# ShuhangGu/DASR

Hardware: NVIDIA B200
Metric: x4 SR output megapixels/sec (RRDBNet-23 G forward) (higher is better)
Workload: dtype bf16

## Files before the change

dasr_b200/csrc/conv_tc2.cu:

```cuda
#include <stdlib.h>
#include "tc_common.cuh"

namespace dasr {

constexpr int TC2_EPI_WARPS = 8;
constexpr int TC2_WARPS = 2 + TC2_EPI_WARPS + 1;
constexpr int TC2_THREADS = 32 * TC2_WARPS;
constexpr int TC2_MAX_STAGES = 6;
constexpr int TC2_MAX_BLOCKS = 6;

struct Tc2Maps {
  CUtensorMap m[8];
};

struct Tc2Args {
  DasrConvTcParams p;
  const float* bias;
  int nchunks;
  int n_half;
  int tiles_x, tiles_y;
  long ntiles;
  int stages, a_stage_bytes, w_bytes;
  int nblk;
  int nb64;
  int nb;
  int acc_stride;
};

template <bool HAS_PRE, int NRES>
__global__ void __cluster_dims__(2, 1, 1) __launch_bounds__(TC2_THREADS, 1)
conv_tc2_kernel(const __grid_constant__ CUtensorMap tmap_in, const __grid_constant__ CUtensorMap tmap_w,
                const __grid_constant__ Tc2Maps em, const Tc2Args a) {
  extern __shared__ __align__(1024) uint8_t smem_raw[];
  uint8_t* smem = reinterpret_cast<uint8_t*>((reinterpret_cast<uintptr_t>(smem_raw) + 1023) & ~uintptr_t(1023));
  uint8_t* sW = smem;
  uint8_t* sA = smem + a.w_bytes;
  uint8_t* sS = sA + (size_t)a.stages * a.a_stage_bytes;
  uint8_t* sR1 = sS + (size_t)a.nblk * EPI_BLK64_BYTES;
  uint8_t* sR2 = sR1 + (NRES >= 1 ? (size_t)a.nblk * EPI_BLK64_BYTES : 0);
  uint64_t* bars = reinterpret_cast<uint64_t*>(sR2 + (NRES >= 2 ? (size_t)a.nblk * EPI_BLK64_BYTES : 0));
  constexpr bool HAS_LOADS = HAS_PRE || NRES > 0;
  uint64_t* full_bar = bars;
  uint64_t* empty_bar = bars + TC2_MAX_STAGES;
  uint64_t* w_bar = bars + 2 * TC2_MAX_STAGES;
  uint64_t* tfull_bar = w_bar + 1;
  uint64_t* tempty_bar = tfull_bar + 2;
  uint64_t* sfull_bar = tempty_bar + 2;
  uint64_t* sfree_bar = sfull_bar + TC2_MAX_BLOCKS;
  uint64_t* pre_bar = sfree_bar + TC2_MAX_BLOCKS;
  uint32_t* tmem_ptr = reinterpret_cast<uint32_t*>(pre_bar + TC2_MAX_BLOCKS);
  float* sBias = reinterpret_cast<float*>(bars + 40);

  const DasrConvTcParams& p = a.p;
  const int warp = threadIdx.x >> 5, lane = threadIdx.x & 31;
  const uint32_t rank = cluster_ctarank();
  const long pair = blockIdx.x >> 1, npairs = gridDim.x >> 1;
  const int cout = p.nt;
  const int co_base = (int)blockIdx.y * p.nt;

  if (threadIdx.x == 0) {
    tma_prefetch_desc(&tmap_in);
    tma_prefetch_desc(&tmap_w);
    tma_prefetch_desc(&em.m[0]);
    for (int s = 0; s < a.stages; s++) {
      mbar_init(&full_bar[s], 1);
      mbar_init(&empty_bar[s], 1);
    }
    mbar_init(w_bar, 1);
    for (int b = 0; b < 2; b++) {
      mbar_init(&tfull_bar[b], 1);
      mbar_init(&tempty_bar[b], 2 * TC2_EPI_WARPS);
    }
    for (int b = 0; b < a.nblk; b++) {
      mbar_init(&sfull_bar[b], TC2_EPI_WARPS);
      mbar_init(&sfree_bar[b], 1);
      mbar_init(&pre_bar[b], 1);
    }
    fence_barrier_init();
  }
  for (int i = threadIdx.x; i < cout; i += TC2_THREADS) sBias[i] = a.bias ? a.bias[co_base + i] : 0.f;
  cluster_sync();
  if (warp == 1) tmem_alloc2(tmem_ptr, 512);
  tc_fence_before();
  __syncthreads();
  tc_fence_after();
  const uint32_t tmem_base = *tmem_ptr;
  pdl_launch_dependents();

  auto tile_of = [&](long it, int& x0, int& y0, int& n) -> bool {
    uint32_t t = 2u * (uint32_t)(pair + it * npairs) + rank;
    const bool live = (long)t < a.ntiles;
    if (p.tile_rev && live) t = (uint32_t)(a.ntiles - 1) - t;
    const uint32_t r = t / (uint32_t)a.tiles_x;
    const uint32_t tx = t - r * (uint32_t)a.tiles_x;
    n = (int)(r / (uint32_t)a.tiles_y);
    const uint32_t ty = r - (uint32_t)n * (uint32_t)a.tiles_y;
    x0 = (int)tx * TILE_W;
    y0 = (int)ty * TILE_H;
    return live;
  };
  const long niter = (a.ntiles / 2 + (a.ntiles & 1) - pair + npairs - 1) / npairs;

  if (warp == 0) {
    if (lane == 0) {
      if (rank == 0) mbar_expect_tx(w_bar, 2u * (uint32_t)a.w_bytes);
      for (int tap = 0; tap < 9; tap++)
        for (int c = 0; c < a.nchunks; c++) {
          const int slot = tap * a.nchunks + c;
          const int row = slot * p.cout + co_base + (int)rank * a.n_half;
          tma2_load_2d(sW + (size_t)slot * a.n_half * ROW_B, &tmap_w, w_bar, 0, row);
        }
      pdl_wait();
      int stage = 0;
      uint32_t phase = 0;
      for (long it = 0; it < niter; it++) {
        int x0, y0, n;
        tile_of(it, x0, y0, n);
        for (int c = 0; c < a.nchunks; c++) {
          mbar_wait(&empty_bar[stage], phase ^ 1);
          if (rank == 0) mbar_expect_tx(&full_bar[stage], 2u * A_HALO_BYTES);
          tma2_load_4d(sA + (size_t)stage * a.a_stage_bytes, &tmap_in, &full_bar[stage],
                       p.nchunk_list ? p.chunk_off[c] : p.in_coff + c * CHUNK, x0 - 1, y0 - 1, n);
          if (++stage == a.stages) { stage = 0; phase ^= 1; }
        }
      }
    }
    __syncwarp();
  } else if (warp == 1) {
    if (rank == 0) {
      const uint32_t idesc = make_idesc_16(256, cout, p.f16);
      const uint32_t a_sbo = (uint32_t)(HALO_W * ROW_B);
      const uint64_t a_hi = ((uint64_t)((a_sbo >> 4) & 0x3FFF) << 32) | ((uint64_t)1 << 46) | ((uint64_t)4 << 61) | ((uint64_t)1 << 16);
      const uint64_t b_hi = ((uint64_t)(((8 * ROW_B) >> 4) & 0x3FFF) << 32) | ((uint64_t)1 << 46) | ((uint64_t)4 << 61) | ((uint64_t)1 << 16);
      const uint32_t a_lo0 = smem_u32(sA) >> 4;
      const uint32_t a_stage_lo = (uint32_t)a.a_stage_bytes >> 4;
      const uint32_t b_lo0 = smem_u32(sW) >> 4;
      const uint32_t b_slot_lo = (uint32_t)(a.n_half * ROW_B) >> 4;
      uint32_t tap_lo[9];
#pragma unroll
      for (int t = 0; t < 9; t++) tap_lo[t] = (uint32_t)(((t / 3) * HALO_W + (t % 3)) * ROW_B) >> 4;
      mbar_wait(w_bar, 0);
      tc_fence_after();
      int stage = 0;
      uint32_t phase = 0;
      for (long it = 0; it < niter; it++) {
        const int acc = (int)(it & 1);
        mbar_wait(&tempty_bar[acc], ((uint32_t)(it >> 1) & 1) ^ 1);
        tc_fence_after();
        const uint32_t d_tmem = tmem_base + (uint32_t)(acc * a.acc_stride);
        for (int c = 0; c < a.nchunks; c++) {
          mbar_wait(&full_bar[stage], phase);
          tc_fence_after();
          if (elect_one()) {
            const uint32_t a_lo = a_lo0 + (uint32_t)stage * a_stage_lo;
            uint32_t b_lo = b_lo0 + (uint32_t)c * b_slot_lo;
            const uint32_t b_tap_step = (uint32_t)a.nchunks * b_slot_lo;
#pragma unroll
            for (int tap = 0; tap < 9; tap++) {
              const uint32_t al = a_lo + tap_lo[tap];
              umma2_bf16(d_tmem, a_hi | (uint64_t)(al & 0x3FFF), b_hi | (uint64_t)(b_lo & 0x3FFF), idesc, (uint32_t)((c | tap) != 0));
              umma2_bf16(d_tmem, a_hi | (uint64_t)((al + 2) & 0x3FFF), b_hi | (uint64_t)((b_lo + 2) & 0x3FFF), idesc, 1u);
              b_lo += b_tap_step;
            }
            umma2_commit_mc(&empty_bar[stage]);
            if (c == a.nchunks - 1) umma2_commit_mc(&tfull_bar[acc]);
          }
          __syncwarp();
          if (++stage == a.stages) { stage = 0; phase ^= 1; }
        }
      }
    }
  } else if (warp == TC2_WARPS - 1) {
    if (lane == 0) {
      pdl_wait();
      const uint32_t nb = (uint32_t)a.nb, nblk = (uint32_t)a.nblk;
      const uint32_t total = (uint32_t)niter * nb;
      const uint32_t nld = (uint32_t)((HAS_PRE ? 1 : 0) + NRES);
      const bool mask_mode = (NRES >= 1) && (p.mask_c1 > p.mask_c0);
      auto issue_loads = [&](uint32_t k) {
        const uint32_t b = k % nblk;
        int x0, y0, n;
        const uint32_t kt = k / nb;
        tile_of((long)kt, x0, y0, n);
        const int i = (int)(k - kt * nb);
        const int wide = i < a.nb64 ? 1 : 0;
        const int col = co_base + i * 64;
        const bool need_r1 = !mask_mode || (col < p.mask_c1 && col + (wide ? 64 : 32) > p.mask_c0);
        mbar_expect_tx(&pre_bar[b], (nld - (need_r1 ? 0u : 1u)) * (uint32_t)(wide ? EPI_BLK64_BYTES : EPI_BLK32_BYTES));
        if constexpr (HAS_PRE) tma_load_4d(sS + (size_t)b * EPI_BLK64_BYTES, &em.m[wide ? 2 : 3], &pre_bar[b], p.pre_coff + col, x0, y0, n);
        if constexpr (NRES >= 1) {
          if (need_r1) tma_load_4d(sR1 + (size_t)b * EPI_BLK64_BYTES, &em.m[wide ? 4 : 5], &pre_bar[b], p.res1_coff + col, x0, y0, n);
        }
        if constexpr (NRES >= 2) tma_load_4d(sR2 + (size_t)b * EPI_BLK64_BYTES, &em.m[wide ? 6 : 7], &pre_bar[b], p.res2_coff + col, x0, y0, n);
      };
      if constexpr (HAS_LOADS)
        for (uint32_t k = 0; k < nblk && k < total; k++) issue_loads(k);
      auto retire = [&](uint32_t k) {
        if constexpr (HAS_LOADS) {
          if (k + nblk < total) issue_loads(k + nblk);
        } else {
          mbar_arrive(&sfree_bar[k % nblk]);
        }
      };
      int x0 = 0, y0 = 0, n = 0;
      bool live = false;
      uint32_t i = 0;
      for (uint32_t k = 0; k < total; k++) {
        const uint32_t b = k % nblk;
        if (i == 0) live = tile_of((long)(k / nb), x0, y0, n);
        mbar_wait(&sfull_bar[b], (k / nblk) & 1);
        if (live) tma_store_4d(&em.m[(int)i < a.nb64 ? 0 : 1], sS + (size_t)b * EPI_BLK64_BYTES, p.out_coff + co_base + (int)i * 64, x0, y0, n);
        bulk_commit();
        if (k >= 1) {
          asm volatile("cp.async.bulk.wait_group.read 1;" ::: "memory");
          retire(k - 1);
        }
        if (++i == nb) i = 0;
      }
      if (total > 0) {
        bulk_wait_read0();
        retire(total - 1);
      }
      bulk_wait0();
    }
    __syncwarp();
  } else {
    const int ew = warp - 2;
    const int wg = ew >> 2;
    const int q = warp & 3;
    const int m = q * 32 + lane;
    const int sw128 = m & 7, sw64 = (m >> 1) & 3;
    const int act = p.act, f16 = p.f16;
    const float slope = p.slope, alpha = p.alpha;
    const bool scale = alpha != 1.f;
    const uint32_t sS_u = smem_u32(sS), sR1_u = smem_u32(sR1), sR2_u = smem_u32(sR2), sBias_u = smem_u32(sBias);
    const bool has_bias = a.bias != nullptr;
    uint32_t k = 0;
    for (long it = 0; it < niter; it++) {
      const int acc = (int)(it & 1);
      mbar_wait(&tfull_bar[acc], (uint32_t)(it >> 1) & 1);
      tc_fence_after();
      const uint32_t t_addr = tmem_base + ((uint32_t)(q * 32) << 16) + (uint32_t)(acc * a.acc_stride);
      for (int i = 0; i < a.nb; i++, k++) {
        const int b = (int)(k % (uint32_t)a.nblk);
        if constexpr (HAS_LOADS) {
          mbar_wait(&pre_bar[b], (k / (uint32_t)a.nblk) & 1);
        } else {
          if (k >= (uint32_t)a.nblk) mbar_wait(&sfree_bar[b], ((k / (uint32_t)a.nblk) & 1) ^ 1);
// ... 62 lines not shown
#pragma unroll
                for (int j = 0; j < 8; j++) {
                  if (!(ms0[j] > 0)) v[j] *= p.mask_slope;
                  if (!(ms1[j] > 0)) v[8 + j] *= p.mask_slope;
                }
              }
            } else {
              fma_h16x8(v, lds128(bR1 + o0), p.beta1, f16);
              fma_h16x8(v + 8, lds128(bR1 + o1), p.beta1, f16);
            }
          }
          if constexpr (NRES >= 2) {
            fma_h16x8(v, lds128(bR2 + o0), p.beta2, f16);
            fma_h16x8(v + 8, lds128(bR2 + o1), p.beta2, f16);
          }
          uint4 o[2];
          pack_h16x16(v, o, f16);
          sts128(bS + o0, o[0]);
          sts128(bS + o1, o[1]);
        }
        fence_proxy_async();
        __syncwarp();
        if (lane == 0) mbar_arrive(&sfull_bar[b]);
      }
    }
  }

  tc_fence_before();
  cluster_sync();
  if (warp == 1) {
    tc_fence_after();
    tmem_dealloc2(tmem_base, 512);
  }
}

__global__ void __cluster_dims__(2, 1, 1) __launch_bounds__(128, 1) mma2_rate_kernel(int n, int iters, long long* out) {
  extern __shared__ __align__(1024) uint8_t smem_raw[];
  uint8_t* smem = reinterpret_cast<uint8_t*>((reinterpret_cast<uintptr_t>(smem_raw) + 1023) & ~uintptr_t(1023));
  __shared__ uint64_t bar;
  __shared__ uint32_t tptr;
  for (int i = threadIdx.x; i < 48 * 1024 / 4; i += blockDim.x) reinterpret_cast<uint32_t*>(smem)[i] = 0;
  if (threadIdx.x == 0) { mbar_init(&bar, 1); fence_barrier_init(); }
  fence_proxy_async();
  cluster_sync();
  if (threadIdx.x < 32) tmem_alloc2(&tptr, 512);
  tc_fence_before();
  __syncthreads();
  tc_fence_after();
  const uint32_t tb = tptr;
  const uint32_t rank = cluster_ctarank();
  if (threadIdx.x < 32 && rank == 0) {
    const uint32_t idesc = make_idesc_bf16(256, n);
    const uint32_t a0 = smem_u32(smem), b0 = smem_u32(smem + 16384);
    long long t0 = clock64();
    for (int it = 0; it < iters; it++) {
      if (elect_one()) {
#pragma unroll 1
        for (int tap = 0; tap < 9; tap++) {
          uint32_t aa = a0 + (uint32_t)(((tap / 3) * 10 + (tap % 3)) * 64);
#pragma unroll
          for (int k = 0; k < 2; k++)
            umma2_bf16(tb, make_desc_sw64(aa + k * 32, 640), make_desc_sw64(b0 + k * 32, 512), idesc, 1u);
        }
        if (it == iters - 1)
          asm volatile("tcgen05.commit.cta_group::2.mbarrier::arrive::one.shared::cluster.b64 [%0];" ::"r"(smem_u32(&bar)) : "memory");
      }
      __syncwarp();
    }
    mbar_wait(&bar, 0);
    long long t1 = clock64();
    if (threadIdx.x == 0 && blockIdx.x == 0) out[0] = (t1 - t0);
  }
  tc_fence_before();
  cluster_sync();
  if (threadIdx.x < 32) { tc_fence_after(); tmem_dealloc2(tb, 512); }
}

}

using namespace dasr;

extern "C" {

static int tc2_plan(const DasrConvTcParams* p, int has_pre, int nres, int* stages_out, int* nblk_out) {
  const int nchunks = p->cin / CHUNK;
  const long w_bytes = (long)9 * nchunks * (p->nt / 2) * ROW_B;
  const int a_stage = (A_HALO_BYTES + 1023) / 1024 * 1024;
  const int bar_bytes = 40 * 8 + 256 * 4 + 64;
  const int per_blk = (1 + nres) * EPI_BLK64_BYTES;
  (void)has_pre;
  static int force_nblk = -1;
  if (force_nblk < 0) {
    const char* e = getenv("DASR_TC2_NBLK");
    force_nblk = e ? atoi(e) : 0;
  }
  for (int want = 4; want >= 2; want--)
    for (int nblk = TC2_MAX_BLOCKS; nblk >= 2; nblk--) {
      if (force_nblk > 0 && nblk != force_nblk) continue;
      const long avail = (long)SMEM_LIMIT - 1024 - w_bytes - (long)nblk * per_blk - bar_bytes;
      int stages = (int)(avail / a_stage);
      if (stages > TC2_MAX_STAGES) stages = TC2_MAX_STAGES;
      if (stages >= want) {
        *stages_out = stages;
        *nblk_out = nblk;
        return 1;
      }
    }
  return 0;
}

int dasr_conv_tc2_supported(const DasrConvTcParams* p) {
  if (!p) return 0;
  if (p->nvar != 1 || p->ntaps != 9 || p->out_mul != 1 || p->epi_mode != 0 || p->a_mode != 0) return 0;
  if (p->nt % 32 != 0 || p->nt < 32 || p->nt > 256 || p->cout % p->nt != 0 || p->cin % CHUNK != 0 || p->cin <= 0) return 0;
  int st, nb;
  const int nres = (p->res1_cs > 0 ? 1 : 0) + (p->res2_cs > 0 ? 1 : 0);
  return tc2_plan(p, p->pre_cs > 0 ? 1 : 0, nres, &st, &nb);
}

int dasr_conv_tc2(const void* in, const void* w, const float* bias, const void* pre, const void* res1, const void* res2,
                  void* out, const DasrConvTcParams* p, void* stream) {
  DASR_REQUIRE(p && in && w && out, "conv_tc2: null argument");
  DASR_REQUIRE(p->nvar == 1 && p->ntaps == 9 && p->out_mul == 1 && p->epi_mode == 0 && p->a_mode == 0,
               "conv_tc2: plain 3x3 geometry with the staged epilogue only");
  DASR_REQUIRE(p->nt % 32 == 0 && p->nt >= 32 && p->nt <= 256 && p->cout % p->nt == 0,
               "conv_tc2: the Cout tile nt must be a multiple of 32 in [32, 256] that divides cout (nt=%d cout=%d)", p->nt, p->cout);
  DASR_REQUIRE(p->N > 0 && p->H > 0 && p->W > 0, "conv_tc2: bad dims");
  DASR_REQUIRE((long)p->N * cdiv(p->W, TILE_W) * cdiv(p->H, TILE_H) < (1L << 30), "conv_tc2: too many tiles for 32-bit tile arithmetic");
  DASR_REQUIRE(p->cin > 0 && p->cin % CHUNK == 0, "conv_tc2: cin must be a multiple of 32 (got %d)", p->cin);
  if (p->nchunk_list > 0) {
    DASR_REQUIRE(p->nchunk_list <= 8 && p->nchunk_list * CHUNK == p->cin, "conv_tc2: chunk list must cover cin");
    for (int i = 0; i < p->nchunk_list; i++)
      DASR_REQUIRE(p->chunk_off[i] >= 0 && p->chunk_off[i] % 8 == 0 && p->chunk_off[i] + CHUNK <= p->in_cs, "conv_tc2: chunk_off[%d]", i);
  } else {
    DASR_REQUIRE(p->in_cs % 8 == 0 && p->in_coff % 8 == 0 && p->in_coff + p->cin <= p->in_cs, "conv_tc2: input slice");
  }
  DASR_REQUIRE(p->out_cs % 8 == 0 && p->out_coff % 8 == 0 && p->out_coff + p->cout <= p->out_cs, "conv_tc2: output slice");
  DASR_REQUIRE(p->act_cols % 16 == 0, "conv_tc2: act_cols must be a multiple of 16");
  DASR_REQUIRE(!(res2 && !res1), "conv_tc2: res2 without res1");
  if (p->mask_c1 > p->mask_c0)
    DASR_REQUIRE(res1 && !res2 && p->mask_c0 % 16 == 0 && p->mask_c1 % 16 == 0 && p->mask_c1 <= p->cout,
                 "conv_tc2: mask mode takes the activation as res1 (no res2) and a range of whole 16-channel groups");
  if (pre) DASR_REQUIRE(p->pre_cs % 8 == 0 && p->pre_coff % 8 == 0 && p->pre_coff + p->cout <= p->pre_cs, "conv_tc2: pre slice");
  if (res1) DASR_REQUIRE(p->res1_cs % 8 == 0 && p->res1_coff % 8 == 0 && p->res1_coff + p->cout <= p->res1_cs, "conv_tc2: res1 slice");
  if (res2) DASR_REQUIRE(p->res2_cs % 8 == 0 && p->res2_coff % 8 == 0 && p->res2_coff + p->cout <= p->res2_cs, "conv_tc2: res2 slice");
  PFN_encodeTiled enc = get_encode();
  if (!enc) {
    set_error("conv_tc2: cuTensorMapEncodeTiled not available");
    return DASR_E_NODRIVER;
  }
  const int has_pre = pre ? 1 : 0, nres = (res1 ? 1 : 0) + (res2 ? 1 : 0);
  Tc2Args a;
  a.p = *p;
  a.bias = bias;
  a.nchunks = p->cin / CHUNK;
  a.n_half = p->nt / 2;
  a.tiles_x = cdiv(p->W, TILE_W);
  a.tiles_y = cdiv(p->H, TILE_H);
  a.ntiles = (long)p->N * a.tiles_x * a.tiles_y;
  a.w_bytes = 9 * a.nchunks * a.n_half * ROW_B;
  a.a_stage_bytes = (A_HALO_BYTES + 1023) / 1024 * 1024;
  a.nb64 = p->nt / 64;
  a.nb = a.nb64 + ((p->nt & 32) ? 1 : 0);
  a.acc_stride = 256;
  const int bar_bytes = 40 * 8 + 256 * 4 + 64;
  int stages = 0, nblk = 0;
  if (!tc2_plan(p, has_pre, nres, &stages, &nblk)) {
    set_error("conv_tc2: filters (%d B per CTA) + %d epilogue block arrays do not fit shared memory", a.w_bytes, 1 + nres);
    return DASR_E_SMEM;
  }
  a.stages = stages;
  a.nblk = nblk;
  size_t smem = 1024 + (size_t)a.w_bytes + (size_t)stages * a.a_stage_bytes + (size_t)nblk * (1 + nres) * EPI_BLK64_BYTES + bar_bytes;
  if (smem < 120 * 1024) smem = 120 * 1024;

  CUtensorMap tm_in, tm_w;
  Tc2Maps em;
  {
    cuuint64_t gdim[4] = {(cuuint64_t)p->in_cs, (cuuint64_t)p->W, (cuuint64_t)p->H, (cuuint64_t)p->N};
    cuuint64_t gstr[3] = {(cuuint64_t)p->in_cs * 2, (cuuint64_t)p->W * p->in_cs * 2, (cuuint64_t)p->H * p->W * p->in_cs * 2};
    cuuint32_t box[4] = {CHUNK, HALO_W, HALO_H, 1};
    cuuint32_t estr[4] = {1, 1, 1, 1};
    CUresult r = enc(&tm_in, CU_TENSOR_MAP_DATA_TYPE_BFLOAT16, 4, const_cast<void*>(in), gdim, gstr, box, estr,
                     CU_TENSOR_MAP_INTERLEAVE_NONE, CU_TENSOR_MAP_SWIZZLE_64B,
                     p->in_cs > CHUNK ? CU_TENSOR_MAP_L2_PROMOTION_L2_64B : CU_TENSOR_MAP_L2_PROMOTION_L2_128B,
                     CU_TENSOR_MAP_FLOAT_OOB_FILL_NONE);
    if (r != CUDA_SUCCESS) { set_error("conv_tc2: cuTensorMapEncodeTiled(input) failed: %d", (int)r); return DASR_E_LAUNCH; }
  }
  {
    cuuint64_t rows = (cuuint64_t)9 * a.nchunks * p->cout;
    cuuint64_t gdim[2] = {CHUNK, rows};
    cuuint64_t gstr[1] = {ROW_B};
    cuuint32_t box[2] = {CHUNK, (cuuint32_t)a.n_half};
    cuuint32_t estr[2] = {1, 1};
    CUresult r = enc(&tm_w, CU_TENSOR_MAP_DATA_TYPE_BFLOAT16, 2, const_cast<void*>(w), gdim, gstr, box, estr,
                     CU_TENSOR_MAP_INTERLEAVE_NONE, CU_TENSOR_MAP_SWIZZLE_64B, CU_TENSOR_MAP_L2_PROMOTION_L2_128B,
                     CU_TENSOR_MAP_FLOAT_OOB_FILL_NONE);
    if (r != CUDA_SUCCESS) { set_error("conv_tc2: cuTensorMapEncodeTiled(filter) failed: %d", (int)r); return DASR_E_LAUNCH; }
  }
  {
    const void* bases[4] = {out, pre, res1, res2};
    const int css[4] = {p->out_cs, p->pre_cs, p->res1_cs, p->res2_cs};
    const char* names[4] = {"output", "pre", "res1", "res2"};
    for (int t = 0; t < 4; t++) {
      em.m[2 * t] = em.m[2 * t + 1] = tm_in;
      if (!bases[t]) continue;
      for (int narrow = 0; narrow < 2; narrow++) {
        if (narrow ? !(p->nt & 32) : (a.nb64 == 0)) continue;
        const int width = narrow ? 32 : 64;
        cuuint64_t gdim[4] = {(cuuint64_t)css[t], (cuuint64_t)p->W, (cuuint64_t)p->H, (cuuint64_t)p->N};
        cuuint64_t gstr[3] = {(cuuint64_t)css[t] * 2, (cuuint64_t)p->W * css[t] * 2, (cuuint64_t)p->H * p->W * css[t] * 2};
        cuuint32_t box[4] = {(cuuint32_t)width, TILE_W, TILE_H, 1};
        cuuint32_t estr[4] = {1, 1, 1, 1};
        CUresult r = enc(&em.m[2 * t + narrow], CU_TENSOR_MAP_DATA_TYPE_BFLOAT16, 4, const_cast<void*>(bases[t]), gdim, gstr, box, estr,
                         CU_TENSOR_MAP_INTERLEAVE_NONE, narrow ? CU_TENSOR_MAP_SWIZZLE_64B : CU_TENSOR_MAP_SWIZZLE_128B,
                         (narrow && css[t] > 32) ? CU_TENSOR_MAP_L2_PROMOTION_L2_64B : CU_TENSOR_MAP_L2_PROMOTION_L2_128B,
                         CU_TENSOR_MAP_FLOAT_OOB_FILL_NONE);
        if (r != CUDA_SUCCESS) { set_error("conv_tc2: cuTensorMapEncodeTiled(%s) failed: %d", names[t], (int)r); return DASR_E_LAUNCH; }
      }
    }
  }
  typedef void (*KernelFn)(const CUtensorMap, const CUtensorMap, const Tc2Maps, const Tc2Args);
  static const KernelFn kernels[6] = {conv_tc2_kernel<false, 0>, conv_tc2_kernel<false, 1>, conv_tc2_kernel<false, 2>,
                                      conv_tc2_kernel<true, 0>,  conv_tc2_kernel<true, 1>,  conv_tc2_kernel<true, 2>};
  const int ki = has_pre * 3 + nres;
  static bool attr_set[6] = {false, false, false, false, false, false};
  if (!attr_set[ki]) {
    cudaError_t e = cudaFuncSetAttribute(kernels[ki], cudaFuncAttributeMaxDynamicSharedMemorySize, SMEM_LIMIT);
    if (e != cudaSuccess) { set_error("conv_tc2: cudaFuncSetAttribute: %s", cudaGetErrorString(e)); return DASR_E_LAUNCH; }
    attr_set[ki] = true;
  }
  long npairs = (a.ntiles + 1) / 2;
  int gx = num_sms() & ~1;
  if ((long)gx > 2 * npairs) gx = (int)(2 * npairs);
  cudaLaunchConfig_t cfg = {};
  cfg.gridDim = dim3(gx, p->cout / p->nt, 1);
  cfg.blockDim = dim3(TC2_THREADS, 1, 1);
  cfg.dynamicSmemBytes = smem;
  cfg.stream = (cudaStream_t)stream;
  cudaLaunchAttribute attrs[1];
  attrs[0].id = cudaLaunchAttributeProgrammaticStreamSerialization;
  attrs[0].val.programmaticStreamSerializationAllowed = pdl_enabled() ? 1 : 0;
  cfg.attrs = attrs;
  cfg.numAttrs = 1;
  cudaError_t e = cudaLaunchKernelEx(&cfg, kernels[ki], tm_in, tm_w, em, a);
  if (e != cudaSuccess) {
    set_error("conv_tc2: launch failed: %s", cudaGetErrorString(e));
    return DASR_E_LAUNCH;
  }
  return check_launch("conv_tc2");
}

int dasr_probe_mma2_rate(int n, int iters, double* cycles_per_mma) {
  long long* d;
  if (cudaMalloc(&d, 8) != cudaSuccess) return DASR_E_LAUNCH;
  cudaFuncSetAttribute(mma2_rate_kernel, cudaFuncAttributeMaxDynamicSharedMemorySize, 64 * 1024);
  mma2_rate_kernel<<<num_sms() & ~1, 128, 64 * 1024>>>(n, iters, d);
  long long h = 0;
  cudaError_t e = cudaMemcpy(&h, d, 8, cudaMemcpyDeviceToHost);
  cudaFree(d);
  if (e != cudaSuccess) { set_error("probe mma2: %s", cudaGetErrorString(e)); return DASR_E_LAUNCH; }
  *cycles_per_mma = (double)h / ((double)iters * 18.0);
  return DASR_OK;
}

}
```

dasr_b200/csrc/selftest.cu:

```cuda
#include <cuda_runtime.h>
#include <cuda_bf16.h>
#include <cuda_fp16.h>
#include <math.h>
#include <stdio.h>
#include <stdlib.h>
#include <string.h>
#include <vector>
#include "../../include/dasr_b200.h"

#define CK(x)                                                                      \
  do {                                                                             \
    cudaError_t e_ = (x);                                                          \
    if (e_ != cudaSuccess) {                                                       \
      printf("CUDA error %s at %s:%d\n", cudaGetErrorString(e_), __FILE__, __LINE__); \
      exit(2);                                                                     \
    }                                                                              \
  } while (0)

extern "C" int dasr_probe_mma_rate(int n, int sbo, int iters, int a_step, double* cycles_per_mma);
extern "C" int dasr_probe_tma_rate(int row_elems, int rows_per_box, int cs, int store, double* cycles_per_box);
extern "C" int dasr_probe_mma2_rate(int n, int iters, double* cycles_per_mma);
static unsigned long long rng_state = 0x1234567ULL;
static inline unsigned rnd() {
  rng_state = rng_state * 6364136223846793005ULL + 1442695040888963407ULL;
  return (unsigned)(rng_state >> 33);
}
static inline float rnd_q(int range, float denom) { return (float)((int)(rnd() % (2 * range + 1)) - range) / denom; }

static int g_fail = 0;
static void report(const char* name, double maxerr, double tol) {
  bool ok = maxerr <= tol;
  printf("[%s] %-58s max_err=%.3e tol=%.1e\n", ok ? "PASS" : "FAIL", name, maxerr, tol);
  if (!ok) g_fail++;
}

template <typename T> static T* dalloc(size_t n) { T* p; CK(cudaMalloc(&p, n * sizeof(T))); CK(cudaMemset(p, 0, n * sizeof(T))); return p; }
template <typename T> static void h2d(T* d, const std::vector<T>& h) { CK(cudaMemcpy(d, h.data(), h.size() * sizeof(T), cudaMemcpyHostToDevice)); }
template <typename T> static std::vector<T> d2h(const T* d, size_t n) { std::vector<T> h(n); CK(cudaMemcpy(h.data(), d, n * sizeof(T), cudaMemcpyDeviceToHost)); return h; }

static void cpu_conv(const std::vector<float>& in, int N, int H, int W, int cin, int in_cs, int in_coff,
                     const std::vector<float>& w, const std::vector<float>* bias, int cout, int kh, int kw, int stride,
                     int pad, int ups, int OH, int OW, std::vector<double>& out) {
  out.assign((size_t)N * OH * OW * cout, 0.0);
  for (int n = 0; n < N; n++)
    for (int oy = 0; oy < OH; oy++)
      for (int ox = 0; ox < OW; ox++)
        for (int co = 0; co < cout; co++) {
          double s = bias ? (*bias)[co] : 0.0;
          for (int dy = 0; dy < kh; dy++)
            for (int dx = 0; dx < kw; dx++) {
              int ty = oy * stride - pad + dy, tx = ox * stride - pad + dx;
              if (ty < 0 || tx < 0 || ty >= H * ups || tx >= W * ups) continue;
              int iy = ty / ups, ix = tx / ups;
              for (int ci = 0; ci < cin; ci++)
                s += (double)in[((size_t)(n * H + iy) * W + ix) * in_cs + in_coff + ci] *
                     (double)w[((size_t)(co * cin + ci) * kh + dy) * kw + dx];
            }
          out[((size_t)(n * OH + oy) * OW + ox) * cout + co] = s;
        }
}

static int g_math = 0;
static void test_f32(int N, int H, int W, int cin, int cout, int k, int stride, int pad, int ups) {
  char name[160];
  int in_cs = cin + 8, in_coff = 4;
  int OH = (H * ups + 2 * pad - k) / stride + 1, OW = (W * ups + 2 * pad - k) / stride + 1;
  std::vector<float> in((size_t)N * H * W * in_cs), w((size_t)cout * cin * k * k), b(cout);
  for (auto& v : in) v = rnd_q(8, 8.f);
  for (auto& v : w) v = rnd_q(8, 16.f);
  for (auto& v : b) v = rnd_q(8, 8.f);
  std::vector<double> ref;
  cpu_conv(in, N, H, W, cin, in_cs, in_coff, w, &b, cout, k, k, stride, pad, ups, OH, OW, ref);
  float *din = dalloc<float>(in.size()), *dw = dalloc<float>(w.size()), *dwp = dalloc<float>(w.size()),
        *db = dalloc<float>(cout), *dout = dalloc<float>(ref.size());
  h2d(din, in); h2d(dw, w); h2d(db, b);
  DasrConvF32Params p;
  memset(&p, 0, sizeof(p));
  p.math = g_math;
  p.N = N; p.H = H; p.W = W; p.cin = cin; p.in_cs = in_cs; p.in_coff = in_coff; p.OH = OH; p.OW = OW;
  p.cout = cout; p.out_cs = cout; p.out_coff = 0; p.kh = k; p.kw = k; p.stride = stride; p.pad = pad; p.ups = ups;
  p.mode = DASR_CONV_FWD; p.act = DASR_ACT_NONE; p.alpha = 1.f;
  int rc = dasr_pack_filter_f32(dw, dwp, cout, cin, k, k, 0, 0);
  rc |= dasr_conv2d_f32(din, dwp, db, nullptr, nullptr, dout, &p, 0);
  CK(cudaDeviceSynchronize());
  if (rc) printf("  rc=%d err=%s\n", rc, dasr_last_error());
  auto got = d2h(dout, ref.size());
  double me = 0;
  for (size_t i = 0; i < ref.size(); i++) me = fmax(me, fabs(got[i] - ref[i]));
  snprintf(name, sizeof(name), "conv_f32%s fwd N%d %dx%d cin%d cout%d k%d s%d p%d ups%d", g_math == 2 ? " tf32" : g_math == 3 ? " tf32x3" : "", N, H, W, cin, cout, k, stride, pad, ups);
  report(name, me, 1e-4);

  if (ups == 1) {
    std::vector<float> dy((size_t)N * OH * OW * cout);
    for (auto& v : dy) v = rnd_q(8, 8.f);
    std::vector<double> dxref((size_t)N * H * W * cin, 0.0);
    for (int n = 0; n < N; n++)
      for (int oy = 0; oy < OH; oy++)
        for (int ox = 0; ox < OW; ox++)
          for (int co = 0; co < cout; co++) {
            double g = dy[((size_t)(n * OH + oy) * OW + ox) * cout + co];
            for (int dyy = 0; dyy < k; dyy++)
              for (int dxx = 0; dxx < k; dxx++) {
                int iy = oy * stride - pad + dyy, ix = ox * stride - pad + dxx;
                if (iy < 0 || ix < 0 || iy >= H || ix >= W) continue;
// ... 296 lines not shown
  DasrConvTcParams p;
  memset(&p, 0, sizeof(p));
  dasr_conv_tc_setup(&p, kind);
  p.N = N; p.H = H; p.W = W; p.cin = cin; p.in_cs = in_cs; p.in_coff = 0;
  p.cout = cout; p.out_cs = in_cs; p.out_coff = (cout <= 128) ? 64 : 0; p.nt = nt;
  p.act = DASR_ACT_LRELU; p.slope = 0.2f; p.alpha = 1.f; p.a_mode = a_mode; p.act_cols = cout;
  p.epi_mode = (kind == 2 || nt % 32) ? 1 : 0;
  if (kind == 1) dasr_pack_filter_tc(dw, dwp, cin, cout, kind, 0);
  else dasr_pack_filter_tc(dw, dwp, cout, cin, kind, 0);
  int rc = 0;
  for (int i = 0; i < 3; i++) rc |= dasr_conv_tc(din, dwp, db, nullptr, nullptr, nullptr, nullptr, dout, &p, 0);
  cudaError_t e = cudaDeviceSynchronize();
  if (rc || e != cudaSuccess) {
    printf("bench conv_tc cin%d cout%d nt%d kind%d amode%d: rc=%d %s cuda=%s\n", cin, cout, nt, kind, a_mode, rc,
           dasr_last_error(), cudaGetErrorString(e));
    if (e != cudaSuccess) exit(3);
    return;
  }
  cudaEvent_t e0, e1;
  cudaEventCreate(&e0); cudaEventCreate(&e1);
  cudaEventRecord(e0);
  for (int i = 0; i < iters; i++) dasr_conv_tc(din, dwp, db, nullptr, nullptr, nullptr, nullptr, dout, &p, 0);
  cudaEventRecord(e1);
  CK(cudaEventSynchronize(e1));
  float ms; cudaEventElapsedTime(&ms, e0, e1);
  ms /= iters;
  double taps = (kind == 2) ? 9.0 : 9.0;
  double flops = 2.0 * N * H * mul * W * mul * cin * cout * taps;
  printf("bench conv_tc kind%d amode%d %dx%dx%d cin%-3d cout%-3d nt%-3d : %8.3f ms  %7.1f TFLOP/s (algorithmic)\n", kind,
         a_mode, N, H, W, cin, cout, nt, ms, flops / ms * 1e-9);
  cudaFree(din); cudaFree(dout); cudaFree(dw); cudaFree(db); cudaFree(dwp);
}

static void bench_tc_fused(int N, int H, int W, int cin, int cout, int nt, int with_pre, int iters, int in_cs = 0, int out_cs = 0,
                           int pair = 0) {
  const int cs = 256;
  const bool planar = in_cs > 0;
  size_t n = (size_t)N * H * W * (planar ? in_cs : cs);
  __nv_bfloat16* buf = dalloc<__nv_bfloat16>(n);
  __nv_bfloat16* obuf = planar ? dalloc<__nv_bfloat16>((size_t)N * H * W * out_cs) : buf;
  std::vector<float> w((size_t)cout * cin * 9);
  for (auto& v : w) v = rnd_q(4, 64.f);
  float* dw = dalloc<float>(w.size());
  h2d(dw, w);
  void* dwp; CK(cudaMalloc(&dwp, dasr_pack_filter_tc_bytes(cout, cin, 0)));
  DasrConvTcParams p;
  memset(&p, 0, sizeof(p));
  dasr_conv_tc_setup(&p, 0);
  p.N = N; p.H = H; p.W = W; p.cin = cin; p.in_cs = planar ? in_cs : cs; p.in_coff = 0;
  p.cout = cout; p.out_cs = planar ? out_cs : cs; p.out_coff = planar ? 0 : cs - cout; p.nt = nt;
  p.act = DASR_ACT_LRELU; p.slope = 0.2f; p.alpha = 1.f; p.act_cols = 32; p.epi_mode = 0;
  p.pre_cs = p.out_cs; p.pre_coff = p.out_coff;
  if (getenv("EPI1") && !with_pre) p.epi_mode = 1;
  dasr_pack_filter_tc(dw, dwp, cout, cin, 0, 0);
  void* pre = with_pre ? (void*)obuf : nullptr;
  int rc = 0;
  auto run = [&]() {
    return pair ? dasr_conv_tc2(buf, dwp, nullptr, pre, nullptr, nullptr, obuf, &p, 0)
                : dasr_conv_tc(buf, dwp, nullptr, pre, nullptr, nullptr, nullptr, obuf, &p, 0);
  };
  for (int i = 0; i < 3; i++) rc |= run();
  cudaError_t e = cudaDeviceSynchronize();
  if (rc || e != cudaSuccess) {
    printf("bench fused cin%d cout%d nt%d: rc=%d %s cuda=%s\n", cin, cout, nt, rc, dasr_last_error(), cudaGetErrorString(e));
    if (e != cudaSuccess) exit(3);
    return;
  }
  cudaEvent_t e0, e1;
  cudaEventCreate(&e0); cudaEventCreate(&e1);
  cudaEventRecord(e0);
  for (int i = 0; i < iters; i++) run();
  cudaEventRecord(e1);
  CK(cudaEventSynchronize(e1));
  float ms; cudaEventElapsedTime(&ms, e0, e1);
  ms /= iters;
  double tiles_per_sm = (double)N * (H / 16) * (W / 8) / 148.0 * (cout / nt);
  if (pair) tiles_per_sm = (double)N * (H / 16) * (W / 8) / 148.0;
  printf("bench fused  %dx%dx%d K%-3d N%-3d nt%-3d pre%d %s%s: %8.3f ms  %7.1f TFLOP/s  %6.2f us/tile\n", N, H, W, cin, cout, nt,
         with_pre, planar ? "planar " : "", pair ? "pair " : "", ms, 2.0 * N * H * W * cin * cout * 9 / ms * 1e-9, ms * 1e3 / tiles_per_sm);
  if (planar) cudaFree(obuf);
  cudaFree(buf); cudaFree(dw); cudaFree(dwp);
}

static void bench_f32(int N, int H, int W, int cin, int cout, int iters) {
  size_t in_n = (size_t)N * H * W * cin, out_n = (size_t)N * H * W * cout;
  float *din = dalloc<float>(in_n), *dout = dalloc<float>(out_n), *dw = dalloc<float>((size_t)9 * cin * cout), *db = dalloc<float>(cout);
  DasrConvF32Params p;
  memset(&p, 0, sizeof(p));
  p.N = N; p.H = H; p.W = W; p.cin = cin; p.in_cs = cin; p.OH = H; p.OW = W; p.cout = cout; p.out_cs = cout;
  p.kh = p.kw = 3; p.stride = 1; p.pad = 1; p.ups = 1; p.alpha = 1.f;
  for (int i = 0; i < 2; i++) dasr_conv2d_f32(din, dw, db, nullptr, nullptr, dout, &p, 0);
  CK(cudaDeviceSynchronize());
  cudaEvent_t e0, e1;
  cudaEventCreate(&e0); cudaEventCreate(&e1);
  cudaEventRecord(e0);
  for (int i = 0; i < iters; i++) dasr_conv2d_f32(din, dw, db, nullptr, nullptr, dout, &p, 0);
  cudaEventRecord(e1);
  CK(cudaEventSynchronize(e1));
  float ms; cudaEventElapsedTime(&ms, e0, e1);
  ms /= iters;
  printf("bench conv_f32 %dx%dx%d cin%-3d cout%-3d : %8.3f ms  %7.2f TFLOP/s\n", N, H, W, cin, cout, ms,
         2.0 * N * H * W * cin * cout * 9 / ms * 1e-9);
  cudaFree(din); cudaFree(dout); cudaFree(dw); cudaFree(db);
}

int main(int argc, char** argv) {
  bool do_check = argc == 1, do_bench = argc == 1;
  for (int i = 1; i < argc; i++) {
    if (!strcmp(argv[i], "check")) do_check = true;
    if (!strcmp(argv[i], "bench")) do_bench = true;
    if (!strcmp(argv[i], "tmarate")) {
      for (int store = 0; store <= 1; store++)
        for (int re : {32, 64, 128, 256})
          for (int cs : {256, 0}) {
            const int rows = 128;
            if ((long)re * 2 * rows > 49152) continue;
            const int pitch = cs ? cs : re;
            double c = 0;
            int rc = dasr_probe_tma_rate(re, rows, pitch, store, &c);
            printf("tma_%s row=%4d B rows/box=%3d pitch=%4d B : %8.1f cycles/box  %6.2f cycles/row  %6.2f B/clk/SM rc=%d\n",
                   store ? "store" : "load ", re * 2, rows, pitch * 2, c, c / rows, re * 2.0 * rows / c, rc);
          }
      return 0;
    }
    if (!strcmp(argv[i], "mmarate")) {
      int ns[] = {32, 64, 96, 128, 192, 256};
      for (int nowait = 0; nowait <= 1; nowait++)
        for (int nacc : {1, 2, 4})
          for (int n : ns) {
            if (n * nacc > 512) continue;
            double c = 0;
            int rc = dasr_probe_mma_rate(n, 640, 200, 64 | (nacc << 16) | (nowait << 20), &c);
            printf("mma_rate M128 N%-3d K16 accumulators=%d %s : %7.1f cycles/MMA  (N/2=%d) rc=%d\n", n, nacc,
                   nowait ? "back-to-back" : "wait/18     ", c, n / 2, rc);
          }
      return 0;
    }
    if (!strcmp(argv[i], "mma2rate")) {
      for (int n : {64, 96, 128, 160, 192, 256}) {
        double c = 0;
        int rc = dasr_probe_mma2_rate(n, 200, &c);
        printf("mma2_rate M256 N%-3d K16 cta_group::2 back-to-back : %7.1f cycles/MMA  (%.1f per 128-pixel tile) rc=%d %s\n", n, c, c / 2,
               rc, rc ? dasr_last_error() : "");
      }
      return 0;
    }
    if (!strcmp(argv[i], "fused")) {
      bench_tc_fused(16, 256, 256, 64, 192, 96, 0, 10);
      bench_tc_fused(16, 256, 256, 32, 160, 160, 1, 10);
      bench_tc_fused(16, 256, 256, 32, 160, 160, 0, 10);
      bench_tc_fused(16, 256, 256, 32, 128, 128, 1, 10);
      bench_tc_fused(16, 256, 256, 32, 96, 96, 1, 10);
      bench_tc_fused(16, 256, 256, 32, 64, 64, 1, 10);
      bench_tc_fused(16, 256, 256, 32, 64, 64, 0, 10);
      bench_tc_fused(2, 256, 256, 32, 64, 64, 1, 40);
      bench_tc_fused(2, 256, 256, 32, 64, 64, 0, 40);
      bench_tc_fused(16, 256, 256, 64, 64, 64, 1, 10);
      bench_tc_fused(16, 256, 256, 64, 64, 64, 0, 10);
      bench_tc_fused(2, 256, 256, 64, 64, 64, 0, 40);
      bench_tc_fused(16, 256, 256, 32, 64, 64, 1, 10, 32, 64);
      bench_tc_fused(16, 256, 256, 32, 64, 64, 0, 10, 32, 64);
      bench_tc_fused(16, 256, 256, 64, 64, 64, 1, 10, 64, 64);
      bench_tc_fused(16, 256, 256, 32, 128, 128, 1, 10, 32, 128);
      bench_tc_fused(16, 256, 256, 64, 192, 96, 0, 10, 64, 192);
      bench_tc_fused(16, 256, 256, 64, 192, 192, 0, 10, 0, 0, 1);
      bench_tc_fused(16, 256, 256, 64, 192, 192, 0, 10, 64, 192, 1);
      bench_tc_fused(16, 256, 256, 32, 128, 128, 0, 10, 0, 0, 1);
      bench_tc_fused(16, 256, 256, 32, 64, 64, 1, 10, 0, 0, 1);
      bench_tc_fused(16, 256, 256, 32, 64, 64, 0, 10, 0, 0, 1);
      bench_tc_fused(16, 256, 256, 64, 64, 64, 1, 10, 0, 0, 1);
      bench_tc_fused(16, 256, 256, 96, 64, 64, 1, 10, 0, 0, 1);
      bench_tc_fused(16, 256, 256, 96, 128, 128, 1, 10, 0, 0, 1);
      bench_tc_fused(16, 256, 256, 64, 128, 128, 1, 10, 0, 0, 1);
      bench_tc_fused(16, 256, 256, 32, 32, 32, 1, 10, 0, 0, 1);
      bench_tc_fused(16, 256, 256, 32, 32, 32, 1, 10, 0, 0, 0);
      bench_tc_fused(16, 256, 256, 128, 64, 64, 1, 10, 0, 0, 1);
      return 0;
    }
    if (!strcmp(argv[i], "prof")) {
      bench_tc(16, 256, 256, 64, 32, 32, 0, 0, 1);
      bench_tc(16, 256, 256, 160, 32, 32, 0, 0, 1);
      bench_tc(16, 256, 256, 32, 192, 192, 1, 0, 1);
      return 0;
    }
  }
  setvbuf(stdout, NULL, _IOLBF, 0);
  cudaDeviceProp prop;
  CK(cudaGetDeviceProperties(&prop, 0));
  printf("device: %s sm_%d%d SMs=%d smem_optin=%zu\n", prop.name, prop.major, prop.minor, prop.multiProcessorCount,
         prop.sharedMemPerBlockOptin);
  if (do_check) {
    for (g_math = 0; g_math <= 3; g_math = g_math ? g_math + 1 : 2) {
      test_f32(2, 9, 11, 3, 64, 3, 1, 1, 1);
      test_f32(2, 8, 8, 32, 32, 3, 1, 1, 1);
      test_f32(1, 7, 5, 64, 3, 3, 1, 1, 1);
      test_f32(2, 12, 10, 9, 64, 4, 2, 1, 1);
      test_f32(1, 9, 9, 16, 20, 4, 1, 1, 1);
      test_f32(1, 6, 7, 16, 16, 3, 1, 1, 2);
      test_f32(1, 8, 8, 8, 1, 4, 1, 1, 1);
      test_f32(1, 10, 10, 12, 8, 5, 1, 2, 1);
      test_f32(2, 16, 16, 64, 128, 4, 2, 1, 1);
      test_f32(2, 9, 9, 64, 1, 4, 1, 1, 1);
      test_f32(1, 11, 7, 30, 2, 3, 1, 1, 1);
    }
    g_math = 0;
    test_wgrad_tc(1, 16, 8, 32, 32);
    test_wgrad_tc(1, 16, 8, 64, 32);
    test_wgrad_tc(2, 20, 13, 96, 32);
    test_wgrad_tc(3, 32, 24, 160, 32);
    test_wgrad_tc(2, 32, 16, 192, 64);
    test_wgrad_tc(1, 48, 40, 64, 64);
    for (int am = 1; am >= 0; am--) {
      test_tc(1, 16, 8, 32, 32, 32, 0, am, 0);
      test_tc(2, 32, 32, 64, 32, 32, 0, am, 0);
      test_tc(1, 20, 13, 96, 32, 32, 0, am, 1);
      test_tc(2, 32, 24, 192, 64, 32, 0, am, 1);
      test_tc(1, 32, 16, 64, 64, 64, 0, am, 1);
      test_tc(1, 20, 13, 96, 32, 32, 0, am, 2);
      test_tc(2, 24, 16, 64, 64, 64, 0, am, 2);
      test_tc(1, 40, 24, 32, 160, 160, 0, am, 2);
      test_tc(1, 19, 11, 64, 192, 96, 0, am, 2);
      test_tc(1, 21, 10, 64, 16, 16, 0, am, 3);
      if (am == 0) {
        test_tc(1, 21, 10, 64, 3, 32, 0, am, 6);
        test_tc(2, 32, 24, 64, 3, 32, 0, am, 6);
        test_tc(1, 16, 8, 32, 1, 32, 0, am, 6);
      }
      test_tc(1, 24, 24, 160, 32, 160, 1, am, 1);
      test_tc(1, 16, 16, 192, 64, 96, 1, am, 0);
      if (am == 0) {
        test_tc(1, 16, 8, 64, 192, 192, 0, 0, 4);
        test_tc(1, 19, 11, 64, 192, 192, 0, 0, 4);
        test_tc(2, 32, 16, 64, 192, 192, 0, 0, 4);
        test_tc(4, 96, 64, 64, 192, 192, 0, 0, 4);
        test_tc(1, 24, 16, 32, 128, 128, 0, 0, 4);
        test_tc(1, 16, 16, 192, 64, 192, 1, 0, 4);
        test_tc(1, 20, 13, 96, 64, 64, 0, 0, 5);
        test_tc(3, 48, 40, 64, 64, 64, 0, 0, 5);
        test_tc(2, 40, 24, 32, 128, 128, 0, 0, 5);
        test_tc(1, 32, 24, 64, 192, 192, 0, 0, 5);
        test_tc(4, 96, 64, 32, 64, 64, 0, 0, 5);
        test_tc(2, 40, 24, 32, 32, 32, 0, 0, 5);
        test_tc(1, 20, 13, 32, 96, 96, 0, 0, 5);
        test_tc(2, 32, 24, 32, 160, 160, 0, 0, 5);
        test_tc(1, 19, 11, 64, 96, 96, 0, 0, 4);
        test_tc(2, 24, 16, 160, 32, 160, 1, 0, 7);
        test_tc(1, 20, 13, 128, 32, 128, 1, 0, 7);
        test_tc(2, 32, 24, 96, 32, 96, 1, 0, 7);
        test_tc(1, 19, 11, 192, 64, 192, 1, 0, 7);
        g_tile_rev = 1;
        test_tc(1, 19, 11, 64, 192, 192, 0, 0, 4);
        test_tc(4, 96, 64, 64, 192, 192, 0, 0, 4);
        test_tc(3, 48, 40, 64, 64, 64, 0, 0, 5);
        test_tc(1, 20, 13, 32, 96, 96, 0, 0, 5);
        g_tile_rev = 0;
        test_tc(1, 16, 8, 64, 128, 64, 0, 0, 4);
        test_tc(2, 24, 16, 64, 128, 32, 0, 0, 5);
        test_tc(1, 20, 13, 96, 192, 96, 0, 0, 4);
        test_tc(1, 16, 16, 512, 64, 32, 0, 0, 4);
// ... 42 lines not shown
```

Measured before the change: 371.0.

## Load 64-channel input chunks per TMA stage with 128B swizzle in tc2 conv

When cin is a multiple of 64 and the chunk offsets are contiguous, the tc2 conv kernel now loads two 32-channel chunks per TMA box with 128B swizzle. The MMA loop issues four K-steps per tap from each stage instead of two, which halves the number of TMA loads and mbarrier round-trips per tile. In exchange each stage is twice as large, so fewer pipeline stages fit in shared memory. A no-MMA probe flag and a matching benchmark are also added to measure load-bound time.

```diff
diff --git a/dasr_b200/csrc/conv_tc2.cu b/dasr_b200/csrc/conv_tc2.cu
--- a/dasr_b200/csrc/conv_tc2.cu
+++ b/dasr_b200/csrc/conv_tc2.cu
@@ -25,6 +25,9 @@
   int nb64;
   int nb;
   int acc_stride;
+  int chunk64;
+  int nloads;
+  int no_mma;
 };
 
 template <bool HAS_PRE, int NRES>
@@ -116,11 +119,12 @@
       for (long it = 0; it < niter; it++) {
         int x0, y0, n;
         tile_of(it, x0, y0, n);
-        for (int c = 0; c < a.nchunks; c++) {
+        for (int c = 0; c < a.nloads; c++) {
           mbar_wait(&empty_bar[stage], phase ^ 1);
-          if (rank == 0) mbar_expect_tx(&full_bar[stage], 2u * A_HALO_BYTES);
+          const int kc = a.chunk64 ? 2 * c : c;
+          if (rank == 0) mbar_expect_tx(&full_bar[stage], 2u * (a.chunk64 ? 2u : 1u) * A_HALO_BYTES);
           tma2_load_4d(sA + (size_t)stage * a.a_stage_bytes, &tmap_in, &full_bar[stage],
-                       p.nchunk_list ? p.chunk_off[c] : p.in_coff + c * CHUNK, x0 - 1, y0 - 1, n);
+                       p.nchunk_list ? p.chunk_off[kc] : p.in_coff + kc * CHUNK, x0 - 1, y0 - 1, n);
           if (++stage == a.stages) { stage = 0; phase ^= 1; }
         }
       }
@@ -129,8 +133,10 @@
   } else if (warp == 1) {
     if (rank == 0) {
       const uint32_t idesc = make_idesc_16(256, cout, p.f16);
-      const uint32_t a_sbo = (uint32_t)(HALO_W * ROW_B);
-      const uint64_t a_hi = ((uint64_t)((a_sbo >> 4) & 0x3FFF) << 32) | ((uint64_t)1 << 46) | ((uint64_t)4 << 61) | ((uint64_t)1 << 16);
+      const uint32_t a_row = a.chunk64 ? 2u * ROW_B : (uint32_t)ROW_B;
+      const uint32_t a_sbo = (uint32_t)HALO_W * a_row;
+      const uint64_t a_hi = ((uint64_t)((a_sbo >> 4) & 0x3FFF) << 32) | ((uint64_t)1 << 46) | ((uint64_t)(a.chunk64 ? 2 : 4) << 61) | ((uint64_t)1 << 16);
+      const int ksteps = a.chunk64 ? 4 : 2;
       const uint64_t b_hi = ((uint64_t)(((8 * ROW_B) >> 4) & 0x3FFF) << 32) | ((uint64_t)1 << 46) | ((uint64_t)4 << 61) | ((uint64_t)1 << 16);
       const uint32_t a_lo0 = smem_u32(sA) >> 4;
       const uint32_t a_stage_lo = (uint32_t)a.a_stage_bytes >> 4;
@@ -138,7 +144,7 @@
       const uint32_t b_slot_lo = (uint32_t)(a.n_half * ROW_B) >> 4;
       uint32_t tap_lo[9];
 #pragma unroll
-      for (int t = 0; t < 9; t++) tap_lo[t] = (uint32_t)(((t / 3) * HALO_W + (t % 3)) * ROW_B) >> 4;
+      for (int t = 0; t < 9; t++) tap_lo[t] = ((uint32_t)((t / 3) * HALO_W + (t % 3)) * a_row) >> 4;
       mbar_wait(w_bar, 0);
       tc_fence_after();
       int stage = 0;
@@ -148,22 +154,31 @@
         mbar_wait(&tempty_bar[acc], ((uint32_t)(it >> 1) & 1) ^ 1);
         tc_fence_after();
         const uint32_t d_tmem = tmem_base + (uint32_t)(acc * a.acc_stride);
-        for (int c = 0; c < a.nchunks; c++) {
+        for (int c = 0; c < a.nloads; c++) {
           mbar_wait(&full_bar[stage], phase);
           tc_fence_after();
           if (elect_one()) {
             const uint32_t a_lo = a_lo0 + (uint32_t)stage * a_stage_lo;
-            uint32_t b_lo = b_lo0 + (uint32_t)c * b_slot_lo;
+            const uint32_t cb = a.chunk64 ? 2u * (uint32_t)c : (uint32_t)c;
+            uint32_t b_lo = b_lo0 + cb * b_slot_lo;
             const uint32_t b_tap_step = (uint32_t)a.nchunks * b_slot_lo;
-#pragma unroll
-            for (int tap = 0; tap < 9; tap++) {
-              const uint32_t al = a_lo + tap_lo[tap];
-              umma2_bf16(d_tmem, a_hi | (uint64_t)(al & 0x3FFF), b_hi | (uint64_t)(b_lo & 0x3FFF), idesc, (uint32_t)((c | tap) != 0));
-              umma2_bf16(d_tmem, a_hi | (uint64_t)((al + 2) & 0x3FFF), b_hi | (uint64_t)((b_lo + 2) & 0x3FFF), idesc, 1u);
-              b_lo += b_tap_step;
+            if (!a.no_mma) {
+#pragma unroll
+              for (int tap = 0; tap < 9; tap++) {
+                const uint32_t al = a_lo + tap_lo[tap];
+#pragma unroll
+                for (int ks = 0; ks < 4; ks++) {
+                  if (ks < ksteps) {
+                    const uint32_t bl = b_lo + (uint32_t)(ks >> 1) * b_slot_lo + 2u * (uint32_t)(ks & 1);
+                    umma2_bf16(d_tmem, a_hi | (uint64_t)((al + 2u * ks) & 0x3FFF), b_hi | (uint64_t)(bl & 0x3FFF), idesc,
+                               (uint32_t)((c | tap | ks) != 0));
+                  }
+                }
+                b_lo += b_tap_step;
+              }
             }
             umma2_commit_mc(&empty_bar[stage]);
-            if (c == a.nchunks - 1) umma2_commit_mc(&tfull_bar[acc]);
+            if (c == a.nloads - 1) umma2_commit_mc(&tfull_bar[acc]);
           }
           __syncwarp();
           if (++stage == a.stages) { stage = 0; phase ^= 1; }
@@ -392,10 +407,26 @@
 
 extern "C" {
 
+static int g_tc2_no_mma = 0;
+
+static int tc2_chunk64(const DasrConvTcParams* p) {
+  static int ok = -1;
+  if (ok < 0) {
+    const char* e = getenv("DASR_TC_CHUNK64");
+    ok = (e && e[0] == '0') ? 0 : 1;
+  }
+  if (!ok || p->cin % (2 * CHUNK) != 0) return 0;
+  if (p->nchunk_list > 0)
+    for (int i = 0; i + 1 < p->nchunk_list; i += 2)
+      if (p->chunk_off[i + 1] != p->chunk_off[i] + CHUNK) return 0;
+  return 1;
+}
+
 static int tc2_plan(const DasrConvTcParams* p, int has_pre, int nres, int* stages_out, int* nblk_out) {
   const int nchunks = p->cin / CHUNK;
   const long w_bytes = (long)9 * nchunks * (p->nt / 2) * ROW_B;
-  const int a_stage = (A_HALO_BYTES + 1023) / 1024 * 1024;
+  const int per_stage = tc2_chunk64(p) ? 2 : 1;
+  const int a_stage = (per_stage * A_HALO_BYTES + 1023) / 1024 * 1024;
   const int bar_bytes = 40 * 8 + 256 * 4 + 64;
   const int per_blk = (1 + nres) * EPI_BLK64_BYTES;
   (void)has_pre;
@@ -410,7 +441,7 @@
       const long avail = (long)SMEM_LIMIT - 1024 - w_bytes - (long)nblk * per_blk - bar_bytes;
       int stages = (int)(avail / a_stage);
       if (stages > TC2_MAX_STAGES) stages = TC2_MAX_STAGES;
-      if (stages >= want) {
+      if (stages >= 2 && stages * per_stage >= want) {
         *stages_out = stages;
         *nblk_out = nblk;
         return 1;
@@ -464,15 +495,18 @@
   a.p = *p;
   a.bias = bias;
   a.nchunks = p->cin / CHUNK;
+  a.chunk64 = tc2_chunk64(p);
+  a.nloads = a.chunk64 ? a.nchunks / 2 : a.nchunks;
   a.n_half = p->nt / 2;
   a.tiles_x = cdiv(p->W, TILE_W);
   a.tiles_y = cdiv(p->H, TILE_H);
   a.ntiles = (long)p->N * a.tiles_x * a.tiles_y;
   a.w_bytes = 9 * a.nchunks * a.n_half * ROW_B;
-  a.a_stage_bytes = (A_HALO_BYTES + 1023) / 1024 * 1024;
+  a.a_stage_bytes = ((a.chunk64 ? 2 : 1) * A_HALO_BYTES + 1023) / 1024 * 1024;
   a.nb64 = p->nt / 64;
   a.nb = a.nb64 + ((p->nt & 32) ? 1 : 0);
   a.acc_stride = 256;
+  a.no_mma = g_tc2_no_mma;
   const int bar_bytes = 40 * 8 + 256 * 4 + 64;
   int stages = 0, nblk = 0;
   if (!tc2_plan(p, has_pre, nres, &stages, &nblk)) {
@@ -489,11 +523,11 @@
   {
     cuuint64_t gdim[4] = {(cuuint64_t)p->in_cs, (cuuint64_t)p->W, (cuuint64_t)p->H, (cuuint64_t)p->N};
     cuuint64_t gstr[3] = {(cuuint64_t)p->in_cs * 2, (cuuint64_t)p->W * p->in_cs * 2, (cuuint64_t)p->H * p->W * p->in_cs * 2};
-    cuuint32_t box[4] = {CHUNK, HALO_W, HALO_H, 1};
+    cuuint32_t box[4] = {(cuuint32_t)(a.chunk64 ? 2 * CHUNK : CHUNK), HALO_W, HALO_H, 1};
     cuuint32_t estr[4] = {1, 1, 1, 1};
     CUresult r = enc(&tm_in, CU_TENSOR_MAP_DATA_TYPE_BFLOAT16, 4, const_cast<void*>(in), gdim, gstr, box, estr,
-                     CU_TENSOR_MAP_INTERLEAVE_NONE, CU_TENSOR_MAP_SWIZZLE_64B,
-                     p->in_cs > CHUNK ? CU_TENSOR_MAP_L2_PROMOTION_L2_64B : CU_TENSOR_MAP_L2_PROMOTION_L2_128B,
+                     CU_TENSOR_MAP_INTERLEAVE_NONE, a.chunk64 ? CU_TENSOR_MAP_SWIZZLE_128B : CU_TENSOR_MAP_SWIZZLE_64B,
+                     (p->in_cs > CHUNK && !a.chunk64) ? CU_TENSOR_MAP_L2_PROMOTION_L2_64B : CU_TENSOR_MAP_L2_PROMOTION_L2_128B,
                      CU_TENSOR_MAP_FLOAT_OOB_FILL_NONE);
     if (r != CUDA_SUCCESS) { set_error("conv_tc2: cuTensorMapEncodeTiled(input) failed: %d", (int)r); return DASR_E_LAUNCH; }
   }
@@ -561,6 +595,8 @@
   return check_launch("conv_tc2");
 }
 
+void dasr_probe_tc2_no_mma(int on) { g_tc2_no_mma = on; }
+
 int dasr_probe_mma2_rate(int n, int iters, double* cycles_per_mma) {
   long long* d;
   if (cudaMalloc(&d, 8) != cudaSuccess) return DASR_E_LAUNCH;
diff --git a/dasr_b200/csrc/selftest.cu b/dasr_b200/csrc/selftest.cu
--- a/dasr_b200/csrc/selftest.cu
+++ b/dasr_b200/csrc/selftest.cu
@@ -20,6 +20,7 @@
 extern "C" int dasr_probe_mma_rate(int n, int sbo, int iters, int a_step, double* cycles_per_mma);
 extern "C" int dasr_probe_tma_rate(int row_elems, int rows_per_box, int cs, int store, double* cycles_per_box);
 extern "C" int dasr_probe_mma2_rate(int n, int iters, double* cycles_per_mma);
+extern "C" void dasr_probe_tc2_no_mma(int on);
 static unsigned long long rng_state = 0x1234567ULL;
 static inline unsigned rnd() {
   rng_state = rng_state * 6364136223846793005ULL + 1442695040888963407ULL;
@@ -482,6 +483,54 @@
   cudaFree(buf); cudaFree(dw); cudaFree(dwp);
 }
 
+static void bench_tc2_launch(int K, int nres, int no_mma, int iters) {
+  const int N = 16, H = 256, W = 256, cs = 256;
+  const size_t n = (size_t)N * H * W * cs;
+  __nv_bfloat16* buf = dalloc<__nv_bfloat16>(n);
+  __nv_bfloat16* buf2 = dalloc<__nv_bfloat16>(n);
+  std::vector<float> w((size_t)64 * K * 9);
+  for (auto& v : w) v = rnd_q(4, 64.f);
+  float* dw = dalloc<float>(w.size());
+  h2d(dw, w);
+  void* dwp; CK(cudaMalloc(&dwp, dasr_pack_filter_tc_bytes(64, K, 0)));
+  dasr_pack_filter_tc(dw, dwp, 64, K, 0, 0);
+  DasrConvTcParams p;
+  memset(&p, 0, sizeof(p));
+  dasr_conv_tc_setup(&p, 0);
+  p.N = N; p.H = H; p.W = W; p.cin = K; p.in_cs = cs; p.in_coff = 64;
+  p.cout = 64; p.nt = 64; p.out_cs = cs; p.act = DASR_ACT_LRELU; p.slope = 0.2f; p.alpha = 1.f; p.epi_mode = 0;
+  void *out, *pre = buf, *res1 = nullptr, *res2 = nullptr;
+  if (K == 64) {
+    out = buf; p.out_coff = p.pre_coff = 128; p.pre_cs = cs; p.act_cols = 32;
+  } else {
+    out = buf2; p.out_coff = 0; p.pre_coff = 192; p.pre_cs = cs; p.act = DASR_ACT_NONE; p.act_cols = 0; p.alpha = 0.2f;
+    res1 = buf; p.res1_cs = cs; p.beta1 = 1.f;
+    if (nres == 2) { res2 = buf2; p.res2_cs = cs; p.res2_coff = 64; p.beta2 = 1.f; }
+  }
+  dasr_probe_tc2_no_mma(no_mma);
+  auto run = [&]() { return dasr_conv_tc2(buf, dwp, nullptr, pre, res1, res2, out, &p, 0); };
+  int rc = 0;
+  for (int i = 0; i < 3; i++) rc |= run();
+  cudaError_t e = cudaDeviceSynchronize();
+  if (rc || e != cudaSuccess) {
+    printf("bench tc2 launch K%d nres%d: rc=%d %s cuda=%s\n", K, nres, rc, dasr_last_error(), cudaGetErrorString(e));
+    dasr_probe_tc2_no_mma(0);
+    if (e != cudaSuccess) exit(3);
+    return;
+  }
+  cudaEvent_t e0, e1;
+  cudaEventCreate(&e0); cudaEventCreate(&e1);
+  cudaEventRecord(e0);
+  for (int i = 0; i < iters; i++) run();
+  cudaEventRecord(e1);
+  CK(cudaEventSynchronize(e1));
+  dasr_probe_tc2_no_mma(0);
+  float ms; cudaEventElapsedTime(&ms, e0, e1);
+  printf("bench tc2 launch%d K%-3d N64 pre%s %-9s: %8.1f us\n", K == 64 ? 3 : 5, K, nres == 2 ? "+res1+res2" : nres ? "+res1     " : "          ",
+         no_mma ? "MMAs off" : "full", ms * 1e3 / iters);
+  cudaFree(buf); cudaFree(buf2); cudaFree(dw); cudaFree(dwp);
+}
+
 static void bench_f32(int N, int H, int W, int cin, int cout, int iters) {
   size_t in_n = (size_t)N * H * W * cin, out_n = (size_t)N * H * W * cout;
   float *din = dalloc<float>(in_n), *dout = dalloc<float>(out_n), *dw = dalloc<float>((size_t)9 * cin * cout), *db = dalloc<float>(cout);
@@ -575,6 +624,14 @@
       bench_tc_fused(16, 256, 256, 32, 32, 32, 1, 10, 0, 0, 1);
       bench_tc_fused(16, 256, 256, 32, 32, 32, 1, 10, 0, 0, 0);
       bench_tc_fused(16, 256, 256, 128, 64, 64, 1, 10, 0, 0, 1);
+      return 0;
+    }
+    if (!strcmp(argv[i], "nomma")) {
+      for (int no_mma = 0; no_mma <= 1; no_mma++) {
+        bench_tc2_launch(64, 0, no_mma, 200);
+        bench_tc2_launch(128, 1, no_mma, 100);
+        bench_tc2_launch(128, 2, no_mma, 100);
+      }
       return 0;
     }
     if (!strcmp(argv[i], "prof")) {
```

Result: no change. 370.6 (median of 6 runs) (-0.1%).
